# rsutormin/KmerGutsJava

Hardware: AMD Instinct MI355X
Metric: amino-acid residues/sec scanned (and hits/sec) on 1 Gbp synthetic, 1/2/4/8 MI355X (higher is better)
Workload: dtype int64; 1 GPU; 1 Gbp contig mix (0.5 kbp..1.024 Mbp, uniform ACGT) on 1 GPU, 6-frame translate + 8-mer lookup vs 1400303159-slot signature table (33.6 GB, load 0.50), -m 5 -g 200; total_bp_rank0=1000000000, contigs_rank0=6351, total_bp_all_ranks=1000000000, num_sigs=1400303159, residues_rank0=1999974596, residues_all_ranks=1999974596, hits_rank0=36744843, hits_all_ranks=36744843, calls_rank0=4, parallelism=contig shards x1, table replicated

## Files before the change

### kmergutsjava_amd/csrc/kg_host_plan.hpp

```cpp
#pragma once

namespace {


template <typename T, T V, T... Vs, typename F>
void dispatch(T x, F &&f)
{
    if constexpr (sizeof...(Vs) == 0) f(std::integral_constant<T, V>{});
    else if (x == V) f(std::integral_constant<T, V>{});
    else dispatch<T, Vs...>(x, f);
}

struct BatchPlan {
    std::vector<uint32_t> ibase;
    uint64_t nblocks = 0, windows = 0, residues = 0;
    uint64_t n_rows = 0, n_cont = 0;
    int64_t longest = 0;
};

template <bool AA>
int plan_batch(const int64_t *offsets, int64_t n_seqs, BatchPlan &b)
{
    constexpr uint32_t PER = AA ? 1 : 6;
    b.ibase.resize((size_t)n_seqs + 1);
    for (int64_t k = 0; k < n_seqs; k++) {
        int64_t L = offsets[k + 1] - offsets[k];
        if (L < 0) return fail(KG_ERR_ARG, "offsets must be non-decreasing");
        b.longest = std::max(b.longest, L);
        if (L > 0xFFFFFFF0ll) return fail(KG_ERR_LIMIT, "a single sequence longer than 2^32-16 characters");
        b.ibase[(size_t)k] = (uint32_t)b.nblocks;
        uint64_t nb;
        if (AA) {
            uint64_t nwin = L >= 9 ? (uint64_t)L - 8 : 0;
            b.windows += nwin;
            b.residues += (uint64_t)L;
            nb = (nwin + kg::kAaWinPerBlock - 1) / kg::kAaWinPerBlock;
        } else {
            uint64_t npos = L >= 24 ? (uint64_t)L - 23 : 0;
            b.windows += 2 * npos;
            for (int f = 0; f < 3; f++)
                if (L - f >= 3) b.residues += 2 * (uint64_t)((L - f) / 3);
            nb = (npos + kg::kDnaPosPerBlock - 1) / kg::kDnaPosPerBlock;
        }
        b.nblocks += nb;
        if (b.nblocks > 0x7FFFFFFFull / PER) return fail(KG_ERR_LIMIT, "batch too large: more than 2^31-1 window rows; split the batch");
    }
    b.ibase[(size_t)n_seqs] = (uint32_t)b.nblocks;
    if (b.windows > 0xFFFFFF00ull) return fail(KG_ERR_LIMIT, "batch too large: more than 2^32-256 windows; split the batch");
    b.n_rows = b.nblocks * PER;
    b.n_cont = (uint64_t)n_seqs * PER;
    return KG_OK;
}

uint64_t bucket_count(uint64_t limit, uint32_t shift) { return (limit + (1ull << shift) - 1) >> shift; }

struct PartPlan {
    bool applicable = false;
    uint32_t shift = 0, buckets = 0;
    uint32_t n_chunks = 0;
    std::vector<uint64_t> clo;
    std::vector<int64_t> cseq;
    uint64_t max_chunk = 0;
    uint32_t n_wg = 0, cap = 0;
    uint64_t n_regions = 0;
    uint32_t ovf_cap = 0;
    uint32_t gshift = 10, groups_stride = 0;
    size_t next_stride = 0;
    size_t scatter_lds = 0;
    bool use_bidx = false, part_counters = false, prog_index = false;
    uint32_t probe_grid = 0, index_grid = 0, verify_grid = 0, lowc_grid = 0, ovf_grid = 0, order_grid = 0;
    uint32_t scatter_prio = 0, index_prio = 0, verify_prio = 0, index_r = 1, probe_grab = 0;
    uint32_t flush_list = 0;
    uint64_t list_slack = 0, ucap = 0, ccap = 0;
    uint32_t n_os = 0;
    bool early_totals = false, place_staged = false, debug = false;
};

template <bool AA>
int plan_partition(const kg_table *t, const BatchPlan &b, bool progress, bool counters_req, PartPlan &pl)
{
    constexpr uint32_t PER = AA ? 1 : 6;
    const uint64_t nblocks = b.nblocks;
    uint32_t shift = env_knob("KG_PART_SHIFT", 21u, 4u, 31u);
    const uint64_t qmax = (uint64_t)KG_MAX_ENCODED / (uint64_t)t->num_sigs + 1;
    while (shift > 4 && qmax >= (1ull << (32 - shift))) shift--;
    while (bucket_count(t->limit, shift) > (uint64_t)kg::kMaxBuckets) shift++;
    while (kg::scatter_lds_bytes<AA>((uint32_t)bucket_count(t->limit, shift)) > 160u * 1024) shift++;
    const bool fits = shift < 32 && qmax < (1ull << (32 - shift)) && nblocks <= (1ull << 23) && t->m35 != 0 &&
                      t->limit < (1ull << 32) - 64;
    const uint32_t mode = env_u32("KG_PARTITION", 2u);
    const bool worth = t->limit >= (64ull << 20) && b.windows >= (1ull << 27);
    if (!(fits && nblocks > 0 && (mode == 1 || (mode == 2 && worth)))) return KG_OK;
    pl.shift = shift;
    pl.buckets = (uint32_t)bucket_count(t->limit, shift);

    constexpr uint32_t WIN = AA ? 64u : 384u;
    uint32_t want = env_u32("KG_PART_CHUNKS", 4u);
    if (want < 1) want = 1;
    if (want > kMaxChunks) want = kMaxChunks;
    if (getenv("KG_PART_MIN_CHUNK_BLOCKS")) {
        const uint64_t min_chunk = std::max(1u, env_u32("KG_PART_MIN_CHUNK_BLOCKS", 600000u));
        while (want > 1 && nblocks / want < min_chunk) want--;
    } else {
        const uint32_t by_size = nblocks < 450000 ? 1u : std::max(2u, (uint32_t)std::lround(std::sqrt((double)nblocks / 325000.0)));
        want = std::min(want, std::max(1u, by_size));
    }
    pl.clo.push_back(0); pl.cseq.push_back(0);
    std::vector<double> cum;
    if (const char *tp = getenv("KG_PART_TAPER")) {
        double acc = 0;
        for (const char *q = tp; *q;) {
            char *endp = nullptr;
            const double v = strtod(q, &endp);
            if (endp == q) break;
            acc += v; cum.push_back(acc);
            q = *endp == ',' ? endp + 1 : endp;
        }
        if (cum.size() >= 2 && cum.size() <= kMaxChunks && acc > 0) { for (auto &x : cum) x /= acc; want = (uint32_t)cum.size(); }
        else cum.clear();
    }
    for (uint32_t c = 1; c < want; c++) {
        const uint64_t target = cum.empty() ? nblocks * c / want : (uint64_t)((double)nblocks * cum[c - 1]);
        const auto it = std::lower_bound(b.ibase.begin(), b.ibase.end(), (uint32_t)target);
        const uint64_t cut = *it;
        if (cut > pl.clo.back() && cut < nblocks) { pl.clo.push_back(cut); pl.cseq.push_back((int64_t)(it - b.ibase.begin())); }
    }
    pl.clo.push_back(nblocks); pl.cseq.push_back((int64_t)b.ibase.size() - 1);
    pl.n_chunks = (uint32_t)pl.clo.size() - 1;
    for (uint32_t c = 0; c < pl.n_chunks; c++) pl.max_chunk = std::max(pl.max_chunk, pl.clo[c + 1] - pl.clo[c]);
    const uint64_t max_chunk = pl.max_chunk;
    const uint64_t chunk_blocks = (max_chunk + kg::kScatterWaves - 1) / kg::kScatterWaves * kg::kScatterWaves;
    const double max_frac = (double)max_chunk / (double)nblocks;
    uint32_t n_wg = env_knob("KG_PART_WGS", 256u, 1u, kMaxGrid);
    if ((uint64_t)n_wg * kg::kScatterWaves > chunk_blocks) n_wg = (uint32_t)((chunk_blocks + kg::kScatterWaves - 1) / kg::kScatterWaves);
    const uint64_t blocks_per_wg = ((chunk_blocks + (uint64_t)n_wg * kg::kScatterWaves - 1) / ((uint64_t)n_wg * kg::kScatterWaves)) * kg::kScatterWaves;
    const double mean = (double)blocks_per_wg * WIN / (double)pl.buckets * (env_u32("KG_PART_SLACK", 100u) / 100.0);
    const uint64_t cap64 = ((uint64_t)(mean + 6.0 * std::sqrt(mean) + 32.0) + 15) / 16 * 16;
    if (cap64 >= (1ull << 24) || (uint64_t)pl.buckets * n_wg >= (1ull << 24)) return KG_OK;
    pl.n_wg = n_wg;
    pl.cap = (uint32_t)cap64;
    pl.n_regions = (uint64_t)pl.buckets * n_wg;
    pl.ovf_cap = env_u32("KG_PART_OVF_GROUPS", (uint32_t)std::min<uint64_t>(1u << 23, std::max<uint64_t>(65536, pl.n_regions * pl.cap / 16 / 8)));
    while (pl.gshift < 12 && ((max_chunk * PER) >> pl.gshift) + 2 > 8192) pl.gshift++;
    pl.groups_stride = (uint32_t)(((max_chunk * PER) >> pl.gshift) + 2);
    if (pl.groups_stride > kg::kMaxGroups) return fail(KG_ERR_LIMIT, "a chunk of the batch holds more than 2^26 window rows");
    pl.next_stride = std::max<size_t>((size_t)pl.buckets + 8, 256);
    pl.use_bidx = t->d_bidx != nullptr && !counters_req && env_u32("KG_BIDX", 1u) != 0;
    pl.part_counters = (counters_req || progress) && !pl.use_bidx;
    pl.prog_index = progress && pl.use_bidx;
    pl.scatter_lds = kg::scatter_lds_bytes<AA>(pl.buckets);
    pl.flush_list = env_knob("KG_SCATTER_FLUSH_LIST", kg::scatter_flush_list_max<AA>(), 1u, kg::scatter_flush_list_max<AA>());
    pl.probe_grid = env_knob("KG_PROBE_GRID", 256u * 8u, 8u, kMaxGrid, 8u);
    pl.index_grid = env_knob("KG_INDEX_GRID", 256u * 4u, 8u, kMaxGrid, 8u);
    pl.scatter_prio = std::min(3u, env_u32("KG_SCATTER_PRIO", 1u));
    pl.index_prio = std::min(3u, env_u32("KG_INDEX_PRIO", 2u));
    pl.verify_prio = std::min(3u, env_u32("KG_VERIFY_PRIO", pl.n_chunks == 1 ? 2u : 0u));
    uint32_t index_r = env_u32("KG_INDEX_R", 0u);
    if (index_r == 0) index_r = mean * 0.7 >= 640.0 ? 1u : mean * 0.7 >= 320.0 ? 2u : 4u;
    if (index_r != 1 && index_r != 2) index_r = 4;
    while (index_r > 1 && (n_wg % index_r != 0 || kg::kIndexN % index_r != 0)) index_r /= 2;
    pl.index_r = index_r;
    pl.verify_grid = env_knob("KG_VERIFY_GRID", 256u * 2u, 1u, kMaxGrid);
    pl.lowc_grid = env_knob("KG_LOWC_GRID", 256u, 1u, kMaxGrid);
    pl.ovf_grid = env_knob("KG_OVF_GRID", 256u, 1u, kMaxGrid);
    pl.list_slack = (uint64_t)(std::max(std::max(pl.probe_grid, pl.index_grid), pl.verify_grid) + 64) * 4 * kg::kUChunk + 4096;
    pl.ucap = ((uint64_t)((double)b.windows * t->stage_ratio * max_frac) + pl.list_slack + kg::kUChunk - 1) / kg::kUChunk * kg::kUChunk;
    pl.ccap = ((uint64_t)((double)b.windows * (t->stage_ratio * 1.25 + 0.03) * max_frac) + pl.list_slack + kg::kUChunk - 1) /
              kg::kUChunk * kg::kUChunk;
    if (test_hook("KG_TEST_TINY_LISTS")) pl.ucap = pl.ccap = kg::kUChunk;
    const uint32_t grab_unit = 256u * (uint32_t)std::max(kg::kProbeN, kg::kIndexN);
    pl.probe_grab = env_knob("KG_PROBE_GRAB", pl.cap, grab_unit, 1u << 24, grab_unit);
    pl.n_os = pl.n_chunks < 2 ? 0u : std::min(env_u32("KG_ORDER_STREAMS", 0u), kMaxOrderStreams);
    pl.early_totals = pl.n_os == 0 && env_u32("KG_EARLY_TOTALS", 1u) != 0;
    pl.order_grid = env_knob("KG_ORDER_GRID", 256u * 3u, 1u, kMaxGrid);
    pl.place_staged = pl.gshift == 10 && env_u32("KG_PLACE_STAGED", 1u) != 0;
    pl.debug = getenv("KG_DEBUG") != nullptr;
    pl.applicable = true;
    return KG_OK;
}

struct DirectPlan {
    uint32_t scan_grid, stage_chunk;
    const uint32_t *d_hbits;
    uint32_t rpg;
    uint64_t stage_cap;
};

template <bool AA>
DirectPlan plan_direct(const kg_table *t, const BatchPlan &b, bool counters)
{
    DirectPlan pl;
    pl.scan_grid = env_knob("KG_SCAN_GRID", 256u * 8u, 1u, kMaxGrid);
    pl.stage_chunk = env_knob("KG_STAGE_CHUNK", 256u, 1u, 1u << 12);
    const uint32_t filter_mode = env_u32("KG_DIRECT_FILTER", 1u);
    pl.d_hbits = (counters || filter_mode == 0 || (filter_mode == 1 && t->limit <= (4ull << 20))) ? nullptr : t->d_hbits;
    pl.rpg = AA ? 1u : env_u32("KG_SCAN_RPG", pl.d_hbits ? 6u : 3u);
    if (pl.rpg != 1 && pl.rpg != 2 && pl.rpg != 3 && pl.rpg != 6) pl.rpg = 3;
    pl.stage_cap = (uint64_t)((double)b.windows * t->stage_ratio) + 4096 + (uint64_t)pl.scan_grid * kg::kWavesPerWG * pl.stage_chunk;
    if (pl.stage_cap > 0xFFFFFF00ull) pl.stage_cap = 0xFFFFFF00ull;
    if (test_hook("KG_TEST_TINY_LISTS")) pl.stage_cap = 256;
    return pl;
}

struct AggPlan {
    uint32_t pshift;
    bool pieces_on;
    uint32_t agg_pairs;
};

AggPlan plan_aggregate()
{
    AggPlan pl;
    pl.pshift = std::min(20u, std::max(6u, env_u32("KG_AGG_BLOCK_SHIFT", 9u)));
    pl.pieces_on = env_u32("KG_AGG_PIECES", 1u) != 0;
    pl.agg_pairs = env_u32("KG_AGG_PAIRS", 1u);
    return pl;
}

}
```

### kmergutsjava_amd/csrc/kg_host_scan.hpp

```cpp
#pragma once

namespace {

struct ScanCtx {
    kg_table *t;
    kg_result *res;
    Scratch &sc;
    const BatchPlan &b;
    const uint8_t *d_seq, *h_seq;
    const int64_t *offsets;
    int64_t n_seqs;
    bool progress, counters;
    bool seq_uploaded;
    uint64_t n_hits = 0;
    int64_t *d_off = nullptr;
    uint32_t *d_ibase = nullptr;
    kg::BlockDesc *d_blocks = nullptr;
    uint32_t *d_counts = nullptr, *d_offs = nullptr, *d_bsb = nullptr;
    uint64_t *d_partial = nullptr, *d_totals = nullptr;
    kg::Progress *d_prog = nullptr;
};

int upload_seq(const ScanCtx &cx, int64_t a, int64_t b)
{
// ... 144 lines not shown
    v.ucur = (unsigned long long *)(pb.d_pc + kPcUcur + c); v.ccur = (unsigned long long *)(pb.d_pc + kPcCcur + c);
    v.base = pb.d_pc + kPcBase + c; v.ctot = pb.d_pc + kPcCtot + c;
    v.ghist = pb.d_ghist + (size_t)c * pl.groups_stride; v.gbase = pb.d_gbase + (size_t)c * (pl.groups_stride + 1);
    v.gcur1 = pb.d_gcur1 + (size_t)c * (kg::kHDigits + 1); v.gcur2 = pb.d_gcur2 + (size_t)c * pl.groups_stride;
    v.gtile = pb.d_gtile + (size_t)c * (kg::kHDigits + 1);
    v.sortA = pb.d_sortA + (uint64_t)c * pb.ucap; v.sortB = pb.d_sortB + (uint64_t)c * pb.ucap;
    return v;
}

int scatter_variant_of(const ScanCtx &cx)
{
    return cx.t->limit >= (uint64_t)cx.t->num_sigs ? 0 : cx.d_prog ? 2 : 1;
}
template <typename F>
void scatter_variant(int variant, F &&f)
{
    if (variant == 0) f(std::false_type{}, std::false_type{});
    else if (variant == 1) f(std::true_type{}, std::false_type{});
    else f(std::true_type{}, std::true_type{});
}

int upload_scatter_cold(const ScanCtx &cx, const PartPlan &pl, const PartBuffers &pb)
{
    kg_table *t = cx.t;
    kg::ScatterCold h[kMaxChunks] = {};
    for (uint32_t c = 0; c < pl.n_chunks; c++) {
        uint32_t *ovfc = pb.d_ovfc + kOvfWords * c;
        h[c].ovf_cursor = ovfc; h[c].ovf_bucket = pb.d_ovf_bucket + (size_t)c * pl.ovf_cap;
        h[c].ovf_ent = pb.d_ovf_ent + (size_t)c * pl.ovf_cap * kg::kGroup;
        h[c].lowc_cursor = ovfc + kOvfLowc; h[c].lowc_blocks = pb.d_lowc + pl.clo[c];
        h[c].ctr = (unsigned long long *)(cx.d_totals + kTotValid); h[c].prog = cx.d_prog;
        h[c].ovf_cap = pl.ovf_cap;
    }
    if (!t->d_cold) HIP_TRY(hipMalloc((void **)&t->d_cold, sizeof h));
    else if (!memcmp(h, t->h_cold, sizeof h)) return KG_OK;
    memcpy(t->h_cold, h, sizeof h);
    HIP_TRY(hipMemcpyAsync(t->d_cold, t->h_cold, sizeof h, hipMemcpyHostToDevice, t->stream));
    return KG_OK;
}

template <bool AA>
int chunk_passes(const ScanCtx &cx, const PartPlan &pl, const PartBuffers &pb, const ChunkView &v)
{
    kg_table *t = cx.t;
    kg::Progress *d_prog = cx.d_prog;
    unsigned long long *d_ctr = (unsigned long long *)(cx.d_totals + kTotValid);
    const hipStream_t s2 = t->stream2, s3 = t->stream3;
    uint32_t *lowc_cursor = v.ovfc + kOvfLowc, *lowc = pb.d_lowc + v.lo;
    const uint32_t limit32 = (uint32_t)std::min<uint64_t>(t->limit, 0xFFFFFFFFull);
    scatter_variant(scatter_variant_of(cx), [&](auto is_short, auto prog) {
        constexpr bool SHORT = decltype(is_short)::value, PROG = decltype(prog)::value;
        hipLaunchKernelGGL((kg::part_scatter_kernel<AA, SHORT, PROG>), dim3(pl.n_wg), dim3(kg::kWave * kg::kScatterWaves), pl.scatter_lds,
                           t->stream, cx.d_seq, cx.d_blocks, v.lo, v.nb, limit32, (uint32_t)t->num_sigs, t->m35, pl.shift, pl.buckets, pl.cap,
                           v.ent, v.fill, t->d_cold + v.c, pl.scatter_prio, pl.flush_list);
    });
    HIP_TRY(hipEventRecord(t->pev[kPevChunk + 2 * v.c], t->stream));
    HIP_TRY(hipStreamWaitEvent(s2, t->pev[kPevChunk + 2 * v.c], 0));
    hipLaunchKernelGGL((kg::lowc_blocks_kernel<AA>), dim3(pl.lowc_grid), dim3(64 * kg::kLowcWaves), 0, s2, cx.d_seq, cx.d_blocks, lowc_cursor, lowc,
                       t->limit, (uint32_t)t->num_sigs, t->m35, pl.shift, pl.n_wg, pl.cap, v.ent, v.fill, v.ovfc, pl.ovf_cap,
                       v.ovf_bucket, v.ovf_ent, d_ctr, d_prog);
    if (pl.use_bidx) {
        const uint32_t tail_start = (uint32_t)std::min<uint64_t>(t->tail_start, 0xFFFFFFFFull);
        dispatch<int, 1, 2, 4>((int)pl.index_r, [&](auto r) {
            dispatch<bool, true, false>(t->bidx_exact, [&](auto exact) {
                dispatch<bool, true, false>(pl.prog_index, [&](auto prog) {
                    constexpr int R = decltype(r)::value;
                    constexpr bool EXACT = decltype(exact)::value, PROG = decltype(prog)::value;
                    hipLaunchKernelGGL((kg::bucket_index_kernel<kg::kIndexN, R, EXACT, PROG>), dim3(pl.index_grid), dim3(256), 0, s2,
                                       t->d_bidx, tail_start, v.ent, v.fill, pl.n_wg, pl.cap, pl.buckets, pl.shift, pl.probe_grab, v.next,
                                       v.cand, v.candused, v.ccur, pb.ccap, d_ctr, pl.index_prio, PROG ? d_prog : (kg::Progress *)nullptr);
                });
            });
        });
    } else {
        dispatch<bool, true, false>(pl.part_counters, [&](auto counters) {
            constexpr bool COUNTERS = decltype(counters)::value;
            hipLaunchKernelGGL((kg::bucket_tag_kernel<COUNTERS>), dim3(pl.probe_grid), dim3(256), 0, s2, t->d_tags, t->limit,
                               (uint64_t)t->num_sigs, v.ent, v.fill, pl.n_wg, pl.cap, pl.buckets, pl.shift, pl.probe_grab, v.next, v.cand,
                               v.candused, v.ccur, pb.ccap, d_ctr, COUNTERS ? d_prog : (kg::Progress *)nullptr);
        });
    }
    HIP_TRY(hipEventRecord(t->pev[kPevChunk + 2 * v.c + 1], s2));
    HIP_TRY(hipStreamWaitEvent(s3, t->pev[kPevChunk + 2 * v.c + 1], 0));
    dispatch<int, 1, 2, 0>(pl.part_counters ? 1 : pl.prog_index ? 2 : 0, [&](auto walks) {
        constexpr bool COUNTERS = decltype(walks)::value == 1, PROG = decltype(walks)::value == 2;
        hipLaunchKernelGGL((kg::verify_kernel<AA, COUNTERS, PROG>), dim3(pl.verify_grid), dim3(256), 0, s3, t->d_entries, t->d_tags, t->limit,
                           (uint64_t)t->num_sigs, t->magic, v.cand, v.candused, v.ccur, pb.ccap, v.ulist, v.cused, v.ucur, pb.ucap, d_ctr,
                           d_prog, pl.verify_prio);
        hipLaunchKernelGGL((kg::overflow_probe_kernel<AA, COUNTERS, PROG>), dim3(pl.ovf_grid), dim3(256), 0, s3, t->d_entries, t->d_tags,
                           t->limit, (uint64_t)t->num_sigs, t->magic, v.ovf_bucket, v.ovf_ent, v.ovfc, pl.ovf_cap, pl.shift, v.ulist,
                           v.cused, v.ucur, pb.ucap, d_ctr, d_prog);
    });
    HIP_TRY(hipEventRecord(t->pev[kPevVerified + v.c], s3));
    HIP_TRY(hipGetLastError());
    return KG_OK;
}

template <bool AA>
int chunk_order(const ScanCtx &cx, const PartPlan &pl, const PartBuffers &pb, const ChunkView &v, uint64_t hits_cap)
{
    constexpr uint32_t PER = AA ? 1 : 6;
    kg_table *t = cx.t;
    kg_result *res = cx.res;
    const uint32_t c = v.c, gshift = pl.gshift;
    const bool last = c + 1 == pl.n_chunks;
    hipStream_t s = t->stream;
    if (pl.n_os) {
        s = t->ostream[c % pl.n_os];
        HIP_TRY(hipStreamWaitEvent(s, t->ev[kEvScattered], 0));
    }
    HIP_TRY(hipStreamWaitEvent(s, t->pev[kPevVerified + c], 0));
    const uint64_t row_lo = (uint64_t)v.lo * PER, row_hi = row_lo + (uint64_t)v.nb * PER;
    const uint32_t g0 = (uint32_t)(row_lo >> gshift);
    const uint32_t n_groups = v.nb ? (uint32_t)(((row_hi - 1) >> gshift) - g0 + 1) : 1u;
    hipLaunchKernelGGL(kg::hit_hist_kernel, dim3(pl.order_grid), dim3(kg::kHThreads), (size_t)n_groups * 4, s, v.ulist, v.cused, v.ucur, pb.ucap,
                       g0, 6u + gshift, n_groups, v.ghist);
    hipLaunchKernelGGL(kg::group_scan_kernel, dim3(1), dim3(kg::kGsThreads), 0, s, v.ghist, n_groups, v.gbase, v.gcur1, v.gcur2, v.ctot, v.gtile);
    if (pl.n_os && c) HIP_TRY(hipStreamWaitEvent(s, t->pev[kPevBase + c - 1], 0));
    hipLaunchKernelGGL(kg::chunk_base_kernel, dim3(1), dim3(1), 0, s, v.ctot, v.base, last ? cx.d_totals : (uint64_t *)nullptr);
    if (pl.n_os) HIP_TRY(hipEventRecord(t->pev[kPevBase + c], s));
    if (pl.early_totals && last) {
        int rc;
        if ((rc = send_counters(t, pb.d_pc, pb.d_ovfc, cx.d_totals, s))) return rc;
        HIP_TRY(hipEventRecord(t->pev[kPevTotals], s));
    }
    hipLaunchKernelGGL((kg::hit_partition_kernel<true>), dim3(pl.order_grid), dim3(kg::kHThreads), 0, s, v.ulist, v.cused, v.ucur, pb.ucap,
                       v.gbase, n_groups, g0, 6u + gshift, v.gcur1, v.sortA, pb.ucap, v.gtile);
    hipLaunchKernelGGL((kg::hit_partition_kernel<false>), dim3(pl.order_grid), dim3(kg::kHThreads), 0, s, v.sortA, v.cused, v.ucur, pb.ucap,
                       v.gbase, n_groups, g0, 6u + gshift, v.gcur2, v.sortB, pb.ucap, v.gtile);
    hipLaunchKernelGGL((kg::group_place_kernel<AA>), dim3(std::min(n_groups, 256u * 8u)), dim3(kg::kHThreads),
                       kg::group_place_lds(gshift, pl.place_staged), s,
                       v.sortB, v.gbase, n_groups, g0, gshift, (uint32_t)row_lo, (uint32_t)row_hi, pb.d_geo, (uint64_t)cx.b.n_rows,
                       pl.place_staged ? 1u : 0u, v.base, res->d_hits, hits_cap, cx.d_offs, res->d_hit_slots);
    HIP_TRY(hipGetLastError());
    return KG_OK;
}

template <bool AA>
int part_allocate(ScanCtx &cx, const PartPlan &pl, PartBuffers &pb)
{
    kg_table *t = cx.t;
    Scratch &sc = cx.sc;
    const uint32_t n_chunks = pl.n_chunks, groups_stride = pl.groups_stride;
    int rc;
    if ((rc = sc.get(&pb.d_ent, (size_t)(pl.n_regions * pl.cap * n_chunks)))) return rc;
    if ((rc = sc.get(&pb.d_fill, (size_t)pl.n_regions * n_chunks))) return rc;
    if ((rc = sc.get(&pb.d_ovf_ent, (size_t)pl.ovf_cap * kg::kGroup * n_chunks))) return rc;
    if ((rc = sc.get(&pb.d_ovf_bucket, (size_t)pl.ovf_cap * n_chunks))) return rc;
    if ((rc = sc.get(&pb.d_next, pl.next_stride * n_chunks))) return rc;
    if ((rc = sc.get(&pb.d_ovfc, kOvfWords * kMaxChunks))) return rc;
    if ((rc = sc.get(&pb.d_lowc, (size_t)cx.b.nblocks + 1))) return rc;
    if ((rc = sc.get(&pb.d_geo, (size_t)cx.b.n_rows))) return rc;
    if ((rc = sc.get(&pb.d_ghist, (size_t)groups_stride * n_chunks))) return rc;
    if ((rc = sc.get(&pb.d_gbase, (size_t)(groups_stride + 1) * n_chunks))) return rc;
    if ((rc = sc.get(&pb.d_gcur1, (size_t)(kg::kHDigits + 1) * n_chunks))) return rc;
    if ((rc = sc.get(&pb.d_gcur2, (size_t)groups_stride * n_chunks))) return rc;
    if ((rc = sc.get(&pb.d_gtile, (size_t)(kg::kHDigits + 1) * n_chunks))) return rc;
    if (kg::group_place_lds(pl.gshift, pl.gshift == 10) > t->place_lds[AA ? 1 : 0]) {
        const size_t want_lds = kg::group_place_lds(pl.gshift, pl.gshift == 10);
        HIP_TRY(hipFuncSetAttribute((const void *)kg::group_place_kernel<AA>, hipFuncAttributeMaxDynamicSharedMemorySize, (int)want_lds));
        t->place_lds[AA ? 1 : 0] = want_lds;
    }
    if (groups_stride * 4u > t->hist_lds) {
        HIP_TRY(hipFuncSetAttribute((const void *)kg::hit_hist_kernel, hipFuncAttributeMaxDynamicSharedMemorySize, (int)(groups_stride * 4u)));
        t->hist_lds = groups_stride * 4u;
    }
    if ((rc = sc.get(&pb.d_pc, kPcWords))) return rc;
    const int sv = scatter_variant_of(cx);
    if (t->scatter_lds[AA ? 1 : 0][sv] < pl.scatter_lds) {
        hipError_t e = hipSuccess;
        scatter_variant(sv, [&](auto is_short, auto prog) {
// ... 312 lines not shown
```

### kmergutsjava_amd/csrc/kg_partition.hpp

```cpp
#pragma once

#include "kg_device.hpp"

namespace kg {

constexpr int kMaxBuckets = 1024;
#ifndef KG_PROBE_N
#define KG_PROBE_N 4
#endif
#ifndef KG_SCATTER_WPE
#define KG_SCATTER_WPE 5
#endif
#ifndef KG_TAG_WPE
#define KG_TAG_WPE 8
#endif
#if KG_SCATTER_WPE
#define KG_SCATTER_REGS __attribute__((amdgpu_waves_per_eu(KG_SCATTER_WPE)))
#else
#define KG_SCATTER_REGS
#endif
#if KG_TAG_WPE
#define KG_TAG_REGS __attribute__((amdgpu_waves_per_eu(KG_TAG_WPE)))
#else
#define KG_TAG_REGS
// ... 771 lines not shown
#pragma unroll
                for (int r = 0; r < R; r++) {
                    uint32_t f = fraw[r];
                    asm volatile("; fill first used here" : "+s"(f));
                    n[r] = min(f, cap);
                    nmax = max(nmax, n[r]);
                }
            }
            uint32_t code[N], vmask = 0;
#pragma unroll
            for (int k = 0; k < N; k++) {
                if (c0 + (uint32_t)(k % PER) * 256u + threadIdx.x >= n[k / PER]) ev[k] = kEntInvalid;
                code[k] = 0;
                if (ev[k] != kEntInvalid) {
                    vmask |= 1u << k;
                    code[k] = bidx[bbase | ((uint32_t)ev[k] & smask)];
                }
            }
            uint32_t candm = 0, walkm = 0, wd[N];
#pragma unroll
            for (int k = 0; k < N; k++) wd[k] = s_lut[code[k]];
#pragma unroll
            for (int k = 0; k < N; k++) {
                const uint32_t q = (uint32_t)ev[k] >> shift;
                const uint32_t c = EXACT ? q : q % kBidxClasses;
                const uint32_t listed = (wd[k] >> c) & 1u;
                candm |= listed << k;
                walkm |= (listed & ((wd[k] | all_walk) >> 31)) << k;
                ran_off = ran_off || (((vmask >> k) & 1u) && !listed && (bbase | ((uint32_t)ev[k] & smask)) >= tail_start);
            }
            if (PROG) {
                if (d_lo == d_hi) {
#pragma unroll
                    for (int k = 0; k < N; k++) {
                        const uint32_t h = bbase | ((uint32_t)ev[k] & smask);
                        if ((vmask >> k) & 1u) pmin = min(pmin, h);
                        if (((vmask & ~candm) >> k) & 1u) pmax1 = max(pmax1, h + 1u);
                    }
                } else {
                    for (int k = 0; k < N; k++)
                        if ((vmask >> k) & 1u) progress_note_home(prog, d_lo, d_hi, bbase | ((uint32_t)ev[k] & smask), (candm >> k) & 1u);
                }
            }
#pragma unroll
            for (int k = 0; k < N; k++) {
                const unsigned long long m = __ballot((candm >> k) & 1u);
                if (!m) continue;
                if ((candm >> k) & 1u) {
                    CandRec c;
                    c.home = bbase | ((uint32_t)ev[k] & smask); c.quo = (uint32_t)ev[k] >> shift;
                    c.id = (uint32_t)(ev[k] >> 32); c.walked = ((walkm >> k) & 1u) ? kWalkOn : kScanOn;
                    stage[sfill + (uint32_t)__popcll(m & ((1ull << lane) - 1ull))] = c;
                }
                sfill += (uint32_t)__popcll(m);
                while (sfill >= kStageFlush) {
                    wave_sync();
                    const unsigned long long at = chunk_reserve(u, kStageFlush, cand_used, cand_cursor, cand_cap, lane);
                    if ((uint32_t)lane < kStageFlush) {
                        const ulonglong2 out = *reinterpret_cast<const ulonglong2 *>(stage + lane);
                        if (at != ~0ull) stream_store16(cand + at + (uint32_t)lane, &out);
                    }
                    sfill -= kStageFlush;
                    wave_sync();
                    if ((uint32_t)lane < sfill) {
                        const ulonglong2 rest = *reinterpret_cast<const ulonglong2 *>(stage + kStageFlush + lane);
                        *reinterpret_cast<ulonglong2 *>(stage + lane) = rest;
                    }
                    wave_sync();
                }
            }
        }
        if (PROG && d_lo == d_hi) progress_note_homes(prog, d_lo, pmin, pmax1);
    }
    if (sfill) {
        wave_sync();
        const CandRec out = stage[(uint32_t)lane < sfill ? lane : 0];
        const unsigned long long at = chunk_reserve(u, sfill, cand_used, cand_cursor, cand_cap, lane);
        if (at != ~0ull && (uint32_t)lane < sfill) stream_store16(cand + at + (uint32_t)lane, &out);
    }
    chunk_finish(u, cand_used, cand_cap, lane);
    flush_ran_off(ran_off, ctr, lane);
}

template <bool AA, bool COUNTERS, bool PROG = false>
__global__ __launch_bounds__(256) void verify_kernel(
    const uint8_t *__restrict__ entries, const uint8_t *__restrict__ tags, uint64_t limit, uint64_t num_sigs, uint64_t magic,
    const CandRec *__restrict__ cand, const uint32_t *__restrict__ cand_used, const unsigned long long *cand_cursor,
    uint64_t cand_cap, kg_hit *__restrict__ ulist, uint32_t *__restrict__ chunk_used, unsigned long long *cursor,
    uint64_t ulist_cap, unsigned long long *ctr, Progress *prog ,
    uint32_t prio )
{
    const int lane = threadIdx.x & 63;
    const uint32_t wave_global = __builtin_amdgcn_readfirstlane(blockIdx.x * 4 + (threadIdx.x >> 6));
    const uint32_t n_waves = gridDim.x * 4;
    if (prio) set_wave_prio(prio);
    TableView tab;
    tab.entries = entries; tab.tags = tags; tab.limit = limit; tab.num_sigs = num_sigs; tab.magic = magic; tab.m35 = 0;
    const unsigned long long cur = *cand_cursor;
    const uint32_t n_chunks = (uint32_t)((cur < cand_cap ? cur : cand_cap) / kUChunk);
    unsigned long long ctr_slots = 0;
    bool ran_off = false;
    UListState u;
    u.base = 0; u.used = kUChunk; u.have = false;
    for (uint32_t c = wave_global; c < n_chunks; c += n_waves) {
        const uint32_t used = cand_used[c];
        for (uint32_t k0 = 0; k0 < used; k0 += 64) {
            const bool act = k0 + (uint32_t)lane < used;
            CandRec r;
            r.home = 0; r.quo = 0; r.id = 0; r.walked = 0;
            if (act) {
                const kg_u32x4 cv = __builtin_nontemporal_load(reinterpret_cast<const kg_u32x4 *>(cand + (uint64_t)c * kUChunk + k0 + lane));
                r.home = cv.x; r.quo = cv.y; r.id = cv.z; r.walked = cv.w;
            }
            const uint64_t quo = r.quo, home = r.home;
            const uint64_t val = quo * num_sigs + home;
            uint64_t s = home + (r.walked & kWalkedMask);
            bool found = false;
            Entry e;
            e.key = 0; e.oI = e.avg = e.fI = 0; e.wt = 0.f;
            if (act && (r.walked & kScanOn)) {
#if KG_SCAN_FULL
                if (s < limit) {
                    const uint64_t s1 = s + 1 < limit ? s + 1 : s, s2 = s + 2 < limit ? s + 2 : s;
                    const Entry e0 = load_entry(tab, s);
                    const uint2 k1 = *reinterpret_cast<const uint2 *>(tab.entries + s1 * 24);
                    const uint2 k2 = *reinterpret_cast<const uint2 *>(tab.entries + s2 * 24);
                    const uint32_t vlo = (uint32_t)val, vhi = (uint32_t)(val >> 32);
                    if (e0.key == (int64_t)val) { found = true; e = e0; }
                    else if (s + 1 < limit && k1.x == vlo && k1.y == vhi) { found = true; s += 1; e = load_entry(tab, s); }
                    else if (s + 2 < limit && k2.x == vlo && k2.y == vhi) { found = true; s += 2; e = load_entry(tab, s); }
                    else s += 3;
                }
#endif
                while (!found) {
                    if (s >= limit) { s = limit; ran_off = true; break; }
                    const uint64_t s1 = s + 1 < limit ? s + 1 : s, s2 = s + 2 < limit ? s + 2 : s;
                    const uint2 k0 = *reinterpret_cast<const uint2 *>(tab.entries + s * 24);
                    const uint2 k1 = *reinterpret_cast<const uint2 *>(tab.entries + s1 * 24);
                    const uint2 k2 = *reinterpret_cast<const uint2 *>(tab.entries + s2 * 24);
                    const uint32_t vlo = (uint32_t)val, vhi = (uint32_t)(val >> 32);
                    if (k0.x == vlo && k0.y == vhi) found = true;
                    else if (s + 1 < limit && k1.x == vlo && k1.y == vhi) { found = true; s += 1; }
                    else if (s + 2 < limit && k2.x == vlo && k2.y == vhi) { found = true; s += 2; }
                    if (found) { e = load_entry(tab, s); break; }
                    s += 3;
                }
                if (COUNTERS) {
                    ctr_slots += (s < limit ? s + 1 : limit) - home;
                    if (prog) progress_note_walk(prog, home, s, limit);
                } else if (PROG) {
                    progress_note_walk(prog, home, s, limit);
                }
            } else if (act) {
                if (!(r.walked & kWalkOn)) {
                    e = load_entry(tab, s);
                    found = e.key == (int64_t)val;
                    if (!found) s += 1;
                }
                if (!found) {
                    const uint32_t f = tag_qs(quo, home);
                    for (;;) {
                        if (s >= limit) { s = limit; ran_off = true; break; }
                        const Tags16 x = load_tags(tab.tags + s);
                        bool emp;
                        const int i = first_stop(x, f, &emp);
                        if (i == 16) { s += 16; continue; }
                        s += (uint64_t)i;
                        if (emp) { if (s >= limit) ran_off = true; break; }
                        e = load_entry(tab, s);
                        if (e.key == (int64_t)val) { found = true; break; }
                        s += 1;
                    }
                }
                if (COUNTERS) {
                    ctr_slots += (s < limit ? s + 1 : limit) - home;
                    if (prog) progress_note_walk(prog, home, s, limit);
                } else if (PROG) {
                    progress_note_walk(prog, home, s, limit);
                }
            }
            const unsigned long long m = __ballot(found);
            const uint32_t total = (uint32_t)__popcll(m);
            if (total) {
                const unsigned long long at = chunk_reserve(u, total, chunk_used, cursor, ulist_cap, lane);
                if (at != ~0ull && found) {
                    kg_hit h;
                    h.container = r.id;
                    h.from0InProt = (int32_t)(uint32_t)s;
                    h.oI = e.oI; h.avgOffFromEnd = e.avg; h.fI = e.fI; h.functionWt = e.wt;
                    stream_store_hit(ulist + at + (uint32_t)__popcll(m & ((1ull << lane) - 1ull)), h);
                }
            }
        }
    }
    chunk_finish(u, chunk_used, ulist_cap, lane);
    flush_ran_off(ran_off, ctr, lane);
    if (COUNTERS) {
        for (int off = 32; off > 0; off >>= 1) ctr_slots += __shfl_down(ctr_slots, off);
        if (lane == 0) atomicAdd(&ctr[1], ctr_slots);
    }
}

template <bool AA, bool COUNTERS, bool PROG = false>
__global__ __launch_bounds__(256) void overflow_probe_kernel(
    const uint8_t *__restrict__ entries, const uint8_t *__restrict__ tags, uint64_t limit, uint64_t num_sigs, uint64_t magic,
    const uint32_t *__restrict__ ovf_bucket, const uint64_t *__restrict__ ovf_ent, const uint32_t *__restrict__ ovf_cursor,
    uint32_t ovf_cap, uint32_t shift, kg_hit *__restrict__ ulist, uint32_t *__restrict__ chunk_used, unsigned long long *cursor, uint64_t ulist_cap,
    unsigned long long *ctr, Progress *prog)
{
    const int lane = threadIdx.x & 63;
    const uint32_t wave_global = __builtin_amdgcn_readfirstlane(blockIdx.x * 4 + (threadIdx.x >> 6));
    const uint32_t n_waves = gridDim.x * 4;
    TableView tab;
    tab.entries = entries; tab.tags = tags; tab.limit = limit; tab.num_sigs = num_sigs; tab.magic = magic; tab.m35 = 0;
    unsigned long long ctr_slots = 0;
    bool ran_off = false;
    UListState u;
    u.base = 0; u.used = kUChunk; u.have = false;
    const uint32_t n_groups = min(*ovf_cursor, ovf_cap);
    for (uint32_t g = wave_global; g < n_groups; g += n_waves) {
        const uint32_t b = ovf_bucket[g];
        uint64_t e[1];
        e[0] = lane < (int)kGroup ? ovf_ent[(uint64_t)g * kGroup + lane] : kEntInvalid;
        probe_entries<AA, 1, COUNTERS || PROG>(tab, b, shift, e, ulist, chunk_used, cursor, ulist_cap, u, ctr_slots, ran_off, lane, prog);
    }
    if (lane == 0 && u.have && u.base + kUChunk <= ulist_cap) chunk_used[u.base / kUChunk] = u.used;
    flush_ran_off(ran_off, ctr, lane);
    if (COUNTERS) {
        for (int off = 32; off > 0; off >>= 1) ctr_slots += __shfl_down(ctr_slots, off);
        if (lane == 0) atomicAdd(&ctr[1], ctr_slots);
    }
}

__global__ void chunk_base_kernel(const uint64_t *chunk_total, uint64_t *base, uint64_t *grand_total)
{
    const uint64_t b = base[0] + *chunk_total;
    base[1] = b;
    if (grand_total) *grand_total = b;
}

}
```

Measured before the change: 132.8 billion residues/s.

## Add batched multi-row verify kernel with prefetched candidates for the last chunk

Adds verify_batch_kernel, in which each wave handles K candidate rows per iteration. It issues the first-probe table loads for all rows together and prefetches the next iteration's candidate records, so more memory requests are in flight against the large random-access table. By default K=4 is used only on the last chunk when there is a single chunk (K=1 otherwise), and the grid for that launch can be tuned separately. The cost is more registers and lower occupancy, plus a second copy of the verify logic whose state machine must match the original kernel exactly.

```diff
diff --git a/kmergutsjava_amd/csrc/kg_host_plan.hpp b/kmergutsjava_amd/csrc/kg_host_plan.hpp
--- a/kmergutsjava_amd/csrc/kg_host_plan.hpp
+++ b/kmergutsjava_amd/csrc/kg_host_plan.hpp
@@ -69,12 +69,15 @@
     size_t scatter_lds = 0;
     bool use_bidx = false, part_counters = false, prog_index = false;
     uint32_t probe_grid = 0, index_grid = 0, verify_grid = 0, lowc_grid = 0, ovf_grid = 0, order_grid = 0;
+    uint32_t verify_k = 1, verify_k_last = 1, verify_grid_last = 0;
     uint32_t scatter_prio = 0, index_prio = 0, verify_prio = 0, index_r = 1, probe_grab = 0;
     uint32_t flush_list = 0;
     uint64_t list_slack = 0, ucap = 0, ccap = 0;
     uint32_t n_os = 0;
     bool early_totals = false, place_staged = false, debug = false;
 };
+
+constexpr uint32_t kVerifyK = 1, kVerifyKOneChunk = 4;
 
 template <bool AA>
 int plan_partition(const kg_table *t, const BatchPlan &b, bool progress, bool counters_req, PartPlan &pl)
@@ -161,9 +164,16 @@
     while (index_r > 1 && (n_wg % index_r != 0 || kg::kIndexN % index_r != 0)) index_r /= 2;
     pl.index_r = index_r;
     pl.verify_grid = env_knob("KG_VERIFY_GRID", 256u * 2u, 1u, kMaxGrid);
+    const auto rows_knob = [](const char *name, uint32_t dflt) {
+        const uint32_t k = env_u32(name, 0u);
+        return k == 1 || k == 2 || k == 4 ? k : dflt;
+    };
+    pl.verify_k = rows_knob("KG_VERIFY_K", kVerifyK);
+    pl.verify_k_last = rows_knob("KG_VERIFY_K_LAST", rows_knob("KG_VERIFY_K", pl.n_chunks == 1 ? kVerifyKOneChunk : kVerifyK));
+    pl.verify_grid_last = env_knob("KG_VERIFY_GRID_LAST", pl.verify_grid, 1u, kMaxGrid);
     pl.lowc_grid = env_knob("KG_LOWC_GRID", 256u, 1u, kMaxGrid);
     pl.ovf_grid = env_knob("KG_OVF_GRID", 256u, 1u, kMaxGrid);
-    pl.list_slack = (uint64_t)(std::max(std::max(pl.probe_grid, pl.index_grid), pl.verify_grid) + 64) * 4 * kg::kUChunk + 4096;
+    pl.list_slack = (uint64_t)(std::max(std::max(pl.probe_grid, pl.index_grid), std::max(pl.verify_grid, pl.verify_grid_last)) + 64) * 4 * kg::kUChunk + 4096;
     pl.ucap = ((uint64_t)((double)b.windows * t->stage_ratio * max_frac) + pl.list_slack + kg::kUChunk - 1) / kg::kUChunk * kg::kUChunk;
     pl.ccap = ((uint64_t)((double)b.windows * (t->stage_ratio * 1.25 + 0.03) * max_frac) + pl.list_slack + kg::kUChunk - 1) /
               kg::kUChunk * kg::kUChunk;
diff --git a/kmergutsjava_amd/csrc/kg_host_scan.hpp b/kmergutsjava_amd/csrc/kg_host_scan.hpp
--- a/kmergutsjava_amd/csrc/kg_host_scan.hpp
+++ b/kmergutsjava_amd/csrc/kg_host_scan.hpp
@@ -250,11 +250,22 @@
     }
     HIP_TRY(hipEventRecord(t->pev[kPevChunk + 2 * v.c + 1], s2));
     HIP_TRY(hipStreamWaitEvent(s3, t->pev[kPevChunk + 2 * v.c + 1], 0));
+    const bool last = v.c + 1 == pl.n_chunks;
     dispatch<int, 1, 2, 0>(pl.part_counters ? 1 : pl.prog_index ? 2 : 0, [&](auto walks) {
         constexpr bool COUNTERS = decltype(walks)::value == 1, PROG = decltype(walks)::value == 2;
-        hipLaunchKernelGGL((kg::verify_kernel<AA, COUNTERS, PROG>), dim3(pl.verify_grid), dim3(256), 0, s3, t->d_entries, t->d_tags, t->limit,
-                           (uint64_t)t->num_sigs, t->magic, v.cand, v.candused, v.ccur, pb.ccap, v.ulist, v.cused, v.ucur, pb.ucap, d_ctr,
-                           d_prog, pl.verify_prio);
+        const uint32_t rows = COUNTERS || PROG ? 1u : last ? pl.verify_k_last : pl.verify_k;
+        const uint32_t grid = COUNTERS || PROG || !last ? pl.verify_grid : pl.verify_grid_last;
+        dispatch<int, 4, 2, 1>((int)rows, [&](auto k) {
+            constexpr int K = decltype(k)::value;
+            if constexpr (K == 1)
+                hipLaunchKernelGGL((kg::verify_kernel<AA, COUNTERS, PROG>), dim3(grid), dim3(256), 0, s3, t->d_entries, t->d_tags, t->limit,
+                                   (uint64_t)t->num_sigs, t->magic, v.cand, v.candused, v.ccur, pb.ccap, v.ulist, v.cused, v.ucur, pb.ucap, d_ctr,
+                                   d_prog, pl.verify_prio);
+            else if constexpr (!COUNTERS && !PROG)
+                hipLaunchKernelGGL((kg::verify_batch_kernel<AA, K>), dim3(grid), dim3(256), 0, s3, t->d_entries, t->d_tags, t->limit,
+                                   (uint64_t)t->num_sigs, t->magic, v.cand, v.candused, v.ccur, pb.ccap, v.ulist, v.cused, v.ucur, pb.ucap, d_ctr,
+                                   pl.verify_prio);
+        });
         hipLaunchKernelGGL((kg::overflow_probe_kernel<AA, COUNTERS, PROG>), dim3(pl.ovf_grid), dim3(256), 0, s3, t->d_entries, t->d_tags,
                            t->limit, (uint64_t)t->num_sigs, t->magic, v.ovf_bucket, v.ovf_ent, v.ovfc, pl.ovf_cap, pl.shift, v.ulist,
                            v.cused, v.ucur, pb.ucap, d_ctr, d_prog);
diff --git a/kmergutsjava_amd/csrc/kg_partition.hpp b/kmergutsjava_amd/csrc/kg_partition.hpp
--- a/kmergutsjava_amd/csrc/kg_partition.hpp
+++ b/kmergutsjava_amd/csrc/kg_partition.hpp
@@ -877,6 +877,49 @@
     flush_ran_off(ran_off, ctr, lane);
 }
 
+struct VerifyRest { uint32_t s; bool found, ran_off; Entry e; };
+__device__ __forceinline__ VerifyRest verify_scan_rest(const TableView &tab, uint32_t lim, uint64_t val, uint32_t s)
+{
+    VerifyRest r;
+    r.found = r.ran_off = false;
+    r.e.key = 0; r.e.oI = r.e.avg = r.e.fI = 0; r.e.wt = 0.f;
+    while (!r.found) {
+        if (s >= lim) { s = lim; r.ran_off = true; break; }
+        const uint32_t s1 = s + 1 < lim ? s + 1 : s, s2 = s + 2 < lim ? s + 2 : s;
+        const uint2 k0 = *reinterpret_cast<const uint2 *>(tab.entries + (uint64_t)s * 24);
+        const uint2 k1 = *reinterpret_cast<const uint2 *>(tab.entries + (uint64_t)s1 * 24);
+        const uint2 k2 = *reinterpret_cast<const uint2 *>(tab.entries + (uint64_t)s2 * 24);
+        const uint32_t vlo = (uint32_t)val, vhi = (uint32_t)(val >> 32);
+        if (k0.x == vlo && k0.y == vhi) r.found = true;
+        else if (s + 1 < lim && k1.x == vlo && k1.y == vhi) { r.found = true; s += 1; }
+        else if (s + 2 < lim && k2.x == vlo && k2.y == vhi) { r.found = true; s += 2; }
+        if (r.found) { r.e = load_entry(tab, s); break; }
+        s += 3;
+    }
+    r.s = s;
+    return r;
+}
+__device__ __forceinline__ VerifyRest verify_walk_rest(const TableView &tab, uint32_t lim, uint32_t f, uint64_t val, uint32_t s)
+{
+    VerifyRest r;
+    r.found = r.ran_off = false;
+    r.e.key = 0; r.e.oI = r.e.avg = r.e.fI = 0; r.e.wt = 0.f;
+    for (;;) {
+        if (s >= lim) { s = lim; r.ran_off = true; break; }
+        const Tags16 x = load_tags(tab.tags + s);
+        bool emp;
+        const int i = first_stop(x, f, &emp);
+        if (i == 16) { s += 16; continue; }
+        s += (uint32_t)i;
+        if (emp) { if (s >= lim) r.ran_off = true; break; }
+        r.e = load_entry(tab, s);
+        if (r.e.key == (int64_t)val) { r.found = true; break; }
+        s += 1;
+    }
+    r.s = s;
+    return r;
+}
+
 template <bool AA, bool COUNTERS, bool PROG = false>
 __global__ __launch_bounds__(256) void verify_kernel(
     const uint8_t *__restrict__ entries, const uint8_t *__restrict__ tags, uint64_t limit, uint64_t num_sigs, uint64_t magic,
@@ -996,6 +1039,151 @@
     }
 }
 
+template <bool AA, int K>
+__global__ __launch_bounds__(256) void verify_batch_kernel(
+    const uint8_t *__restrict__ entries, const uint8_t *__restrict__ tags, uint64_t limit, uint64_t num_sigs, uint64_t magic,
+    const CandRec *__restrict__ cand, const uint32_t *__restrict__ cand_used, const unsigned long long *cand_cursor,
+    uint64_t cand_cap, kg_hit *__restrict__ ulist, uint32_t *__restrict__ chunk_used, unsigned long long *cursor,
+    uint64_t ulist_cap, unsigned long long *ctr, uint32_t prio )
+{
+    static_assert(K == 2 || K == 4, "K rows per iteration: a divisor of the chunk's rows");
+    static_assert(kUChunk % (64 * K) == 0, "an iteration stays inside one candidate chunk");
+    enum : uint32_t { kNone = 0, kScan = 1, kFp = 2, kWalk = 3 };
+    enum : uint32_t { kDone = 0, kPayload = 4, kMatch = 5, kScanRest = 6, kWalkRest = 7 };
+    const int lane = threadIdx.x & 63;
+    const uint32_t wave_global = __builtin_amdgcn_readfirstlane(blockIdx.x * 4 + (threadIdx.x >> 6));
+    const uint32_t n_waves = gridDim.x * 4;
+    if (prio) set_wave_prio(prio);
+    TableView tab;
+    tab.entries = entries; tab.tags = tags; tab.limit = limit; tab.num_sigs = num_sigs; tab.magic = magic; tab.m35 = 0;
+    const unsigned long long cur = *cand_cursor;
+    const uint32_t n_chunks = (uint32_t)((cur < cand_cap ? cur : cand_cap) / kUChunk);
+    bool ran_off = false;
+    UListState u;
+    u.base = 0; u.used = kUChunk; u.have = false;
+    const auto request = [&](kg_u32x4 (&v)[K], uint32_t cc, uint32_t kk, uint32_t count, const CandRec *safe) {
+#pragma unroll
+        for (int j = 0; j < K; j++) {
+            const uint32_t i = kk + 64u * (uint32_t)j + (uint32_t)lane;
+            v[j] = __builtin_nontemporal_load(reinterpret_cast<const kg_u32x4 *>(i < count ? cand + (uint64_t)cc * kUChunk + i : safe));
+        }
+    };
+    uint32_t c = wave_global, k0 = 0, used = 0, used_next = 0;
+    kg_u32x4 cv[K];
+    if (c < n_chunks) {
+        used = cand_used[c];
+        if (c + n_waves < n_chunks) used_next = cand_used[c + n_waves];
+        request(cv, c, 0, used, cand + (uint64_t)c * kUChunk);
+    }
+    const uint32_t lim = (uint32_t)limit;
+    while (c < n_chunks) {
+        const CandRec *safe = cand + (uint64_t)c * kUChunk;
+        uint32_t s[K], st[K];
+        uint32_t foundm = 0;
+        kg_u32x4 A[K];
+        kg_u32x2 B[K], C[K], D[K];
+        const auto record = [&](int j, const Entry &e) {
+            A[j].x = (uint32_t)e.key; A[j].y = (uint32_t)((uint64_t)e.key >> 32); A[j].z = (uint32_t)e.oI; A[j].w = (uint32_t)e.avg;
+            B[j].x = (uint32_t)e.fI; B[j].y = __float_as_uint(e.wt);
+        };
+#pragma unroll
+        for (int j = 0; j < K; j++) {
+            const bool act = k0 + 64u * (uint32_t)j + (uint32_t)lane < used;
+            const uint32_t wk = cv[j].w;
+            s[j] = cv[j].x + (wk & kWalkedMask);
+            const bool in = s[j] < lim;
+            st[j] = !act ? kNone : (wk & kScanOn) ? (in ? kScan : kScanRest) : (wk & kWalkOn) ? (in ? kWalk : kWalkRest) : kFp;
+            const bool whole = st[j] == kScan || st[j] == kFp;
+            const uint8_t *pa = whole ? entries + (uint64_t)s[j] * 24 : st[j] == kWalk ? tags + s[j] : reinterpret_cast<const uint8_t *>(safe);
+            const uint8_t *pb = pa + (whole ? 16u : 0u);
+            const uint8_t *pc = pa + (st[j] == kScan && s[j] + 1 < lim ? 24u : 0u);
+            const uint8_t *pd = pa + (st[j] == kScan && s[j] + 2 < lim ? 48u : 0u);
+            __builtin_memcpy(&A[j], pa, 16);
+            __builtin_memcpy(&B[j], pb, 8);
+            __builtin_memcpy(&C[j], pc, 8);
+            __builtin_memcpy(&D[j], pd, 8);
+        }
+        const bool hop = k0 + 64u * K >= used;
+        const uint32_t c_next = hop ? c + n_waves : c, k_next = hop ? 0u : k0 + 64u * K;
+        const uint32_t count_next = c_next < n_chunks ? (hop ? used_next : used) : 0u;
+        kg_u32x4 nv[K];
+        request(nv, c_next, k_next, count_next, safe);
+        if (hop) used_next = c_next < n_chunks && c_next + n_waves < n_chunks ? cand_used[c_next + n_waves] : 0u;
+#pragma unroll
+        for (int j = 0; j < K; j++) {
+            const uint64_t val = (uint64_t)cv[j].y * num_sigs + cv[j].x;
+            const uint32_t vlo = (uint32_t)val, vhi = (uint32_t)(val >> 32);
+            const bool at_s = A[j].x == vlo && A[j].y == vhi;
+            const uint32_t first = st[j];
+            if (first != kScanRest && first != kWalkRest) st[j] = kDone;
+            if (first == kScan) {
+                if (at_s) foundm |= 1u << j;
+                else if (s[j] + 1 < lim && C[j].x == vlo && C[j].y == vhi) { s[j] += 1; st[j] = kPayload; }
+                else if (s[j] + 2 < lim && D[j].x == vlo && D[j].y == vhi) { s[j] += 2; st[j] = kPayload; }
+                else { s[j] += 3; st[j] = kScanRest; }
+            } else if (first == kFp) {
+                if (at_s) foundm |= 1u << j;
+                else { s[j] += 1; st[j] = kWalkRest; }
+            } else if (first == kWalk) {
+                Tags16 x;
+                x.w[0] = A[j].x; x.w[1] = A[j].y; x.w[2] = A[j].z; x.w[3] = A[j].w;
+                bool emp;
+                const int i = first_stop(x, tag_qs(cv[j].y, cv[j].x), &emp);
+                if (i == 16) { s[j] += 16; st[j] = kWalkRest; }
+                else {
+                    s[j] += (uint32_t)i;
+                    if (emp) ran_off = ran_off || s[j] >= lim;
+                    else st[j] = kMatch;
+                }
+            }
+            if (st[j] == kPayload || st[j] == kMatch) {
+                const uint8_t *rec = entries + (uint64_t)s[j] * 24;
+                __builtin_memcpy(&A[j], rec, 16);
+                __builtin_memcpy(&B[j], rec + 16, 8);
+            }
+        }
+#pragma unroll
+        for (int j = 0; j < K; j++) {
+            const uint64_t val = (uint64_t)cv[j].y * num_sigs + cv[j].x;
+            const uint32_t vlo = (uint32_t)val, vhi = (uint32_t)(val >> 32);
+            if (st[j] == kPayload) foundm |= 1u << j;
+            else if (st[j] == kMatch) {
+                if (A[j].x == vlo && A[j].y == vhi) foundm |= 1u << j;
+                else { s[j] += 1; st[j] = kWalkRest; }
+            }
+            if (st[j] == kScanRest || st[j] == kWalkRest) {
+                const VerifyRest r = st[j] == kScanRest ? verify_scan_rest(tab, lim, val, s[j])
+                                                          : verify_walk_rest(tab, lim, tag_qs(cv[j].y, cv[j].x), val, s[j]);
+                s[j] = r.s;
+                if (r.found) { foundm |= 1u << j; record(j, r.e); }
+                ran_off = ran_off || r.ran_off;
+            }
+        }
+#pragma unroll
+        for (int j = 0; j < K; j++) {
+            const bool found = (foundm >> j) & 1u;
+            const unsigned long long m = __ballot(found);
+            const uint32_t total = (uint32_t)__popcll(m);
+            if (total) {
+                const unsigned long long at = chunk_reserve(u, total, chunk_used, cursor, ulist_cap, lane);
+                if (at != ~0ull && found) {
+                    kg_hit h;
+                    h.container = cv[j].z;
+                    h.from0InProt = (int32_t)(uint32_t)s[j];
+                    h.oI = (int32_t)A[j].z; h.avgOffFromEnd = (int32_t)A[j].w; h.fI = (int32_t)B[j].x; h.functionWt = __uint_as_float(B[j].y);
+                    stream_store_hit(ulist + at + __builtin_amdgcn_mbcnt_hi((uint32_t)(m >> 32), __builtin_amdgcn_mbcnt_lo((uint32_t)m, 0u)), h);
+                }
+            }
+        }
+        if (hop) used = count_next;
+        c = c_next; k0 = k_next;
+#pragma unroll
+        for (int j = 0; j < K; j++) cv[j] = nv[j];
+    }
+    chunk_finish(u, chunk_used, ulist_cap, lane);
+    flush_ran_off(ran_off, ctr, lane);
+}
+
 template <bool AA, bool COUNTERS, bool PROG = false>
 __global__ __launch_bounds__(256) void overflow_probe_kernel(
     const uint8_t *__restrict__ entries, const uint8_t *__restrict__ tags, uint64_t limit, uint64_t num_sigs, uint64_t magic,
```

After: 132.9 billion residues/s, median of 4. No clear change (+0.1%).
